# Jiang-Muyun/PointNet12

Hardware: NVIDIA B200
Metric: pointnet2_semseg_forward_points_per_sec (higher is better)
Workload: dtype f32 (MLP products as split bf16 hi/lo on tensor cores)

## Files before the change

### pointnet12_b200/csrc/fps.cu

```cuda
#include <cooperative_groups.h>

#include <type_traits>

#include "common.cuh"
#include "tcgen05.cuh"

namespace cg = cooperative_groups;

namespace pn {

constexpr int kMaxCluster = 16;
constexpr unsigned kNoIndex = 0xFFFFFFFFu;

struct __align__(32) FpsMsg {
    unsigned long long key;
    float x, y, z;
    float pad[3];
};

constexpr int kFpsSmemHeader = 2 * kMaxCluster * (int)sizeof(FpsMsg) + 2 * 32 * (int)sizeof(uint2) + 64;

__device__ __forceinline__ unsigned map_to_cta(unsigned addr, unsigned rank) {
    unsigned r;
    asm volatile("mapa.shared::cluster.u32 %0, %1, %2;" : "=r"(r) : "r"(addr), "r"(rank));
    return r;
}

template <int THREADS, int PTS, bool CLUSTER>
__global__ void __launch_bounds__(THREADS, 1)
fps_kernel(const float* __restrict__ xyz, int64_t sB, int64_t sN, int64_t sC, int N, int npoint,
           const int64_t* __restrict__ start, int64_t* __restrict__ out, unsigned long long* seq, int chunk, int async_x) {
    constexpr int NW = THREADS / 32;
    extern __shared__ __align__(32) unsigned char smem_raw[];
    FpsMsg* cl_slots = reinterpret_cast<FpsMsg*>(smem_raw);
    uint2* warp_slots = reinterpret_cast<uint2*>(smem_raw + 2 * kMaxCluster * sizeof(FpsMsg));
    unsigned long long* xbar = reinterpret_cast<unsigned long long*>(smem_raw + kFpsSmemHeader - 64);
    float* sx = reinterpret_cast<float*>(smem_raw + kFpsSmemHeader);
    float* sy = sx + chunk;
    float* sz = sy + chunk;

    unsigned CL = 1, rank = 0;
    if constexpr (CLUSTER) {
        cg::cluster_group cluster = cg::this_cluster();
        CL = cluster.num_blocks();
        rank = cluster.block_rank();
    }
    const int b = blockIdx.x / CL;
    const float* __restrict__ p = xyz + (int64_t)b * sB;
    const int base = rank * chunk;
    const int tid = threadIdx.x, lane = tid & 31, warp = tid >> 5;

    float x[PTS], y[PTS], z[PTS], d[PTS];
#pragma unroll
    for (int k = 0; k < PTS; ++k) {
        const int li = tid + k * THREADS;
        const int j = base + li;
        const bool ok = li < chunk && j < N;
        x[k] = ok ? p[(int64_t)j * sN] : 0.0f;
        y[k] = ok ? p[(int64_t)j * sN + sC] : 0.0f;
        z[k] = ok ? p[(int64_t)j * sN + 2 * sC] : 0.0f;
        d[k] = ok ? 1e10f : -2.0f;
        if (li < chunk) {
            sx[li] = x[k];
            sy[li] = y[k];
            sz[li] = z[k];
        }
    }
    int far = (int)start[b];
    float cx = p[(int64_t)far * sN], cy = p[(int64_t)far * sN + sC], cz = p[(int64_t)far * sN + 2 * sC];
    if constexpr (CLUSTER) {
        if (async_x && tid == 0) {
            tc::mbar_init(tc::smem_u32(&xbar[0]), 1);
            tc::mbar_init(tc::smem_u32(&xbar[1]), 1);
            tc::mbar_init_fence();
        }
        __syncthreads();
        cg::this_cluster().sync();
    } else {
        __syncthreads();
    }

    int64_t* __restrict__ o = out + (int64_t)b * npoint;
    for (int i = 0; i < npoint; ++i) {
        if (rank == 0 && tid == 0) {
            o[i] = far;
            if (seq) *reinterpret_cast<volatile unsigned long long*>(seq + (int64_t)b * npoint + i) = ((unsigned long long)(unsigned)far << 32) | 1ull;
        }
        float bv = -1.0f;
        int bk = 0;
#pragma unroll
        for (int k = 0; k < PTS; ++k) {
            const float dd = sqdist_diff(x[k], y[k], z[k], cx, cy, cz);
            d[k] = fminf(d[k], dd);
            if (d[k] > bv) {
                bv = d[k];
                bk = k;
            }
        }
        const unsigned vb = __float_as_uint(fmaxf(bv, 0.0f));
        const unsigned gi = bv < 0.0f ? kNoIndex : (unsigned)(base + tid + bk * THREADS);
        const unsigned wm = __reduce_max_sync(0xffffffffu, vb);
        const unsigned wi = __reduce_min_sync(0xffffffffu, vb == wm ? gi : kNoIndex);
        const int par = i & 1;
        unsigned bm, bi;
        if constexpr (NW > 1) {
            if (lane == 0) warp_slots[par * 32 + warp] = make_uint2(wm, wi);
            __syncthreads();
            const uint2 s = lane < NW ? warp_slots[par * 32 + lane] : make_uint2(0u, kNoIndex);
            bm = __reduce_max_sync(0xffffffffu, s.x);
            bi = __reduce_min_sync(0xffffffffu, s.x == bm ? s.y : kNoIndex);
        } else {
            bm = wm;
            bi = wi;
        }
        if constexpr (!CLUSTER) {
            far = (int)bi;
            cx = sx[far];
            cy = sy[far];
            cz = sz[far];
        } else {
            cg::cluster_group cluster = cg::this_cluster();
            if (async_x) {
                const unsigned l_bar = tc::smem_u32(&xbar[par]);
                if (tid == 0) tc::mbar_arrive_expect_tx(l_bar, CL * 20u);
                if (warp == 0 && lane < (int)CL) {
                    const unsigned long long key = ((unsigned long long)bm << 32) | (unsigned long long)(~bi);
                    const int li = bi == kNoIndex ? 0 : (int)bi - base;
                    const unsigned r_slot = map_to_cta(tc::smem_u32(&cl_slots[par * kMaxCluster + rank]), lane);
                    const unsigned r_bar = map_to_cta(l_bar, lane);
                    asm volatile(
                        "st.async.weak.shared::cluster.mbarrier::complete_tx::bytes.v4.b32 [%0], {%1, %2, %3, %4}, [%5];" ::"r"(r_slot),
                        "r"((unsigned)(key & 0xFFFFFFFFull)), "r"((unsigned)(key >> 32)), "r"(__float_as_uint(sx[li])),
                        "r"(__float_as_uint(sy[li])), "r"(r_bar)
                        : "memory");
                    asm volatile("st.async.weak.shared::cluster.mbarrier::complete_tx::bytes.b32 [%0], %1, [%2];" ::"r"(r_slot + 16),
                                 "r"(__float_as_uint(sz[li])), "r"(r_bar)
                                 : "memory");
                }
                tc::mbar_wait(l_bar, (unsigned)((i >> 1) & 1));
            } else {
            if (warp == 0 && lane < (int)CL) {
                FpsMsg m;
                m.key = ((unsigned long long)bm << 32) | (unsigned long long)(~bi);
                const int li = bi == kNoIndex ? 0 : (int)bi - base;
                m.x = sx[li];
                m.y = sy[li];
                m.z = sz[li];
                m.pad[0] = m.pad[1] = m.pad[2] = 0.0f;
                FpsMsg* dst = cluster.map_shared_rank(&cl_slots[par * kMaxCluster + rank], lane);
                *dst = m;
            }
            cluster.sync();
            }
            unsigned long long best = 0ull;
            int bc = 0;
            for (int c = 0; c < (int)CL; ++c) {
                const unsigned long long k = cl_slots[par * kMaxCluster + c].key;
                if (k > best) {
                    best = k;
                    bc = c;
                }
            }
            far = (int)(~(unsigned)(best & 0xFFFFFFFFull));
            const FpsMsg& w = cl_slots[par * kMaxCluster + bc];
            cx = w.x;
            cy = w.y;
            cz = w.z;
        }
    }
    if constexpr (CLUSTER) {
        if (async_x) cg::this_cluster().sync();
    }
}

struct __align__(32) FpsSlot {
    unsigned val, idx;
    float x, y, z;
    float pad[3];
};
constexpr int kMaxSlots = 64;
constexpr int kSlotBytes = 20;
constexpr int kAsyncSmemHeader = 64 + 2 * kMaxSlots * (int)sizeof(FpsSlot);

template <int NW, int PTS, bool ZT>
__global__ void __launch_bounds__(NW * 32, 1)
fps_async_kernel(const float* __restrict__ xyz, int64_t sB, int64_t sN, int64_t sC, int N, int npoint,
                 const int64_t* __restrict__ start, int64_t* __restrict__ out, unsigned long long* seq, int chunk) {
    constexpr int THREADS = NW * 32;
    extern __shared__ __align__(32) unsigned char smem_raw[];
    unsigned long long* mbar = reinterpret_cast<unsigned long long*>(smem_raw);
    FpsSlot* slots = reinterpret_cast<FpsSlot*>(smem_raw + 64);
    float* sx = reinterpret_cast<float*>(smem_raw + kAsyncSmemHeader);
    float* sy = sx + chunk;
    float* sz = sy + chunk;
    float* zt = sz + chunk;

    cg::cluster_group cluster = cg::this_cluster();
    const unsigned CL = cluster.num_blocks();
    const unsigned rank = cluster.block_rank();
    const int nslot = (int)CL * NW;
    const int b = blockIdx.x / CL;
    const float* __restrict__ p = xyz + (int64_t)b * sB;
    const int base = rank * chunk;
    const int tid = threadIdx.x, lane = tid & 31, warp = tid >> 5;

    static_assert(PTS % 2 == 0, "points are processed in packed pairs");
    unsigned long long xp[PTS / 2], yp[PTS / 2], zp[PTS / 2];
    float d[PTS];
#pragma unroll
    for (int k = 0; k < PTS; k += 2) {
        float x[2], y[2], z[2];
#pragma unroll
        for (int u = 0; u < 2; ++u) {
            const int li = tid + (k + u) * THREADS;
            const int j = base + li;
            const bool ok = li < chunk && j < N;
            x[u] = ok ? p[(int64_t)j * sN] : 0.0f;
            y[u] = ok ? p[(int64_t)j * sN + sC] : 0.0f;
            z[u] = ok ? p[(int64_t)j * sN + 2 * sC] : 0.0f;
            d[k + u] = ok ? 1e10f : -2.0f;
            if (li < chunk) {
                sx[li] = x[u];
                sy[li] = y[u];
                sz[li] = z[u];
            }
        }
        xp[k / 2] = pack2(x[0], x[1]);
        yp[k / 2] = pack2(y[0], y[1]);
        zp[k / 2] = pack2(z[0], z[1]);
    }
    if constexpr (ZT) {
        for (int i = tid; i < N; i += THREADS) zt[i] = p[(int64_t)i * sN + 2 * sC];
    }
    if (tid == 0) {
        tc::mbar_init(tc::smem_u32(&mbar[0]), 1);
        tc::mbar_init(tc::smem_u32(&mbar[1]), 1);
        tc::mbar_init_fence();
    }
    int far = (int)start[b];
    far = min(max(far, 0), N - 1);
    float cx = p[(int64_t)far * sN], cy = p[(int64_t)far * sN + sC], cz = p[(int64_t)far * sN + 2 * sC];
    __syncthreads();
    cluster.sync();

    const unsigned my_slot = rank * NW + warp;
    const unsigned dst_cta = lane < (int)CL ? lane : 0;
    const unsigned r_slot0 = map_to_cta(tc::smem_u32(&slots[my_slot]), dst_cta);
    const unsigned r_bar0 = map_to_cta(tc::smem_u32(&mbar[0]), dst_cta);
    const unsigned l_bar0 = tc::smem_u32(&mbar[0]);
    constexpr unsigned kParSlotOff = kMaxSlots * sizeof(FpsSlot), kParBarOff = sizeof(unsigned long long);

    int64_t* __restrict__ o = out + (int64_t)b * npoint;
    for (int i = 0; i < npoint; ++i) {
        const int par = i & 1;
        if (rank == 0 && tid == 0) {
            o[i] = far;
            if (seq) *reinterpret_cast<volatile unsigned long long*>(seq + (int64_t)b * npoint + i) = ((unsigned long long)(unsigned)far << 32) | 1ull;
        }
        if (i == npoint - 1) break;
        if (tid == 0)
            tc::mbar_arrive_expect_tx(l_bar0 + par * kParBarOff, (unsigned)(nslot * (ZT ? 16 : kSlotBytes)));
        float bv = -1.0f;
        int bk = 0;
        const unsigned long long ncx = pack2(-cx, -cx), ncy = pack2(-cy, -cy), ncz = pack2(-cz, -cz);
#pragma unroll
        for (int k = 0; k < PTS; k += 2) {
            float d0, d1;
            sqdist_diff2(xp[k / 2], yp[k / 2], zp[k / 2], ncx, ncy, ncz, d0, d1);
            d[k] = fminf(d[k], d0);
            if (d[k] > bv) {
                bv = d[k];
                bk = k;
            }
            d[k + 1] = fminf(d[k + 1], d1);
            if (d[k + 1] > bv) {
                bv = d[k + 1];
                bk = k + 1;
            }
        }
        const unsigned vb = __float_as_uint(fmaxf(bv, 0.0f));
        const unsigned gi = bv < 0.0f ? kNoIndex : (unsigned)(base + tid + bk * THREADS);
        const unsigned wm = __reduce_max_sync(0xffffffffu, vb);
        const unsigned wi = __reduce_min_sync(0xffffffffu, vb == wm ? gi : kNoIndex);
        if (lane < (int)CL) {
            const int li = wi == kNoIndex ? 0 : (int)wi - base;
            const float mx = sx[li], my = sy[li];
            const unsigned r_slot = r_slot0 + par * kParSlotOff, r_bar = r_bar0 + par * kParBarOff;
            asm volatile(
                "st.async.weak.shared::cluster.mbarrier::complete_tx::bytes.v4.b32 [%0], {%1, %2, %3, %4}, [%5];" ::"r"(
                    r_slot),
                "r"(wm), "r"(wi), "r"(__float_as_uint(mx)), "r"(__float_as_uint(my)), "r"(r_bar)
                : "memory");
            if constexpr (!ZT) {
                const float mz = sz[li];
                asm volatile("st.async.weak.shared::cluster.mbarrier::complete_tx::bytes.b32 [%0], %1, [%2];" ::"r"(
                                 r_slot + 16),
                             "r"(__float_as_uint(mz)), "r"(r_bar)
                             : "memory");
            }
        }
        tc::mbar_wait(l_bar0 + par * kParBarOff, (unsigned)((i >> 1) & 1));
        unsigned sv = 0u, si = kNoIndex;
        float px = 0.f, py = 0.f, pz = 0.f;
        if (lane < nslot) {
            const FpsSlot& s0 = slots[par * kMaxSlots + lane];
            sv = s0.val; si = s0.idx; px = s0.x; py = s0.y;
            if constexpr (!ZT) pz = s0.z;
        }
        if (lane + 32 < nslot) {
            const FpsSlot& s1 = slots[par * kMaxSlots + lane + 32];
            if (s1.val > sv || (s1.val == sv && s1.idx < si)) {
                sv = s1.val; si = s1.idx; px = s1.x; py = s1.y;
                if constexpr (!ZT) pz = s1.z;
            }
        }
        const unsigned bm = __reduce_max_sync(0xffffffffu, sv);
        const unsigned bi = __reduce_min_sync(0xffffffffu, sv == bm ? si : kNoIndex);
        const unsigned who = __ballot_sync(0xffffffffu, sv == bm && si == bi);
        const int src = __ffs(who) - 1;
        far = (int)bi;
        cx = __shfl_sync(0xffffffffu, px, src);
        cy = __shfl_sync(0xffffffffu, py, src);
        if constexpr (ZT) cz = zt[min(bi, (unsigned)(N - 1))];
        else cz = __shfl_sync(0xffffffffu, pz, src);
    }
    cluster.sync();
}

template <int NW, int PTS>
__global__ void __launch_bounds__(NW * 32, NW == 8 ? 2 : 1)
fps_pruned_kernel(const float* __restrict__ xyz, int64_t sB, int64_t sN, int64_t sC, const unsigned char* __restrict__ grid_ws,
                  size_t ws_stride, size_t sorted_off, int N, int npoint, const int64_t* __restrict__ start,
                  int64_t* __restrict__ out, unsigned long long* seq, int no_prune) {
    static_assert(PTS % 2 == 0, "points are processed in packed pairs");
    constexpr int CAP = NW * PTS * 32, NQ = PTS / 2;
    extern __shared__ __align__(32) unsigned char smem_raw[];
    unsigned long long* mbar = reinterpret_cast<unsigned long long*>(smem_raw);
    FpsSlot* slots = reinterpret_cast<FpsSlot*>(smem_raw + 64);
    float4* rec = reinterpret_cast<float4*>(smem_raw + kAsyncSmemHeader);

    cg::cluster_group cluster = cg::this_cluster();
    const unsigned CL = cluster.num_blocks();
    const unsigned rank = cluster.block_rank();
    const int nslot = (int)CL * NW;
    const int b = blockIdx.x / CL;
    const float* __restrict__ p = xyz + (int64_t)b * sB;
    const float4* __restrict__ sorted = reinterpret_cast<const float4*>(grid_ws + (size_t)b * ws_stride + sorted_off);
    const int tid = threadIdx.x, lane = tid & 31, warp = tid >> 5;
    float4* wrec = rec + (size_t)warp * NQ * 2 * 32 + lane;
    const int g0 = (int)rank * CAP + warp * PTS * 32;

    float d[PTS];
    float lo[3] = {3.0e38f, 3.0e38f, 3.0e38f}, hi[3] = {-3.0e38f, -3.0e38f, -3.0e38f};
#pragma unroll
    for (int q = 0; q < NQ; ++q) {
        float4 v[2];
#pragma unroll
        for (int u = 0; u < 2; ++u) {
            const int j = g0 + (2 * q + u) * 32 + lane;
            const bool ok = j < N;
            v[u] = make_float4(0.f, 0.f, 0.f, __int_as_float(-1));
            if (ok) v[u] = sorted[j];
            d[2 * q + u] = ok ? 1e10f : -2.0f;
            if (ok) {
                lo[0] = fminf(lo[0], v[u].x); hi[0] = fmaxf(hi[0], v[u].x);
                lo[1] = fminf(lo[1], v[u].y); hi[1] = fmaxf(hi[1], v[u].y);
                lo[2] = fminf(lo[2], v[u].z); hi[2] = fmaxf(hi[2], v[u].z);
            }
        }
        wrec[(q * 2 + 0) * 32] = make_float4(v[0].x, v[1].x, v[0].y, v[1].y);
        wrec[(q * 2 + 1) * 32] = make_float4(v[0].z, v[1].z, v[0].w, v[1].w);
    }
#pragma unroll
    for (int c = 0; c < 3; ++c)
#pragma unroll
        for (int o = 16; o; o >>= 1) {
            lo[c] = fminf(lo[c], __shfl_xor_sync(0xffffffffu, lo[c], o));
            hi[c] = fmaxf(hi[c], __shfl_xor_sync(0xffffffffu, hi[c], o));
        }
    const bool warp_empty = g0 >= N;
    if (tid == 0) {
        tc::mbar_init(tc::smem_u32(&mbar[0]), 1);
        tc::mbar_init(tc::smem_u32(&mbar[1]), 1);
        tc::mbar_init_fence();
    }
    int far = (int)start[b];
    far = min(max(far, 0), N - 1);
    float cx = p[(int64_t)far * sN], cy = p[(int64_t)far * sN + sC], cz = p[(int64_t)far * sN + 2 * sC];
    __syncthreads();
    cluster.sync();

    const unsigned my_slot = rank * NW + warp;
    const unsigned dst_cta = lane < (int)CL ? lane : 0;
    const unsigned r_slot0 = map_to_cta(tc::smem_u32(&slots[my_slot]), dst_cta);
    const unsigned r_bar0 = map_to_cta(tc::smem_u32(&mbar[0]), dst_cta);
    const unsigned l_bar0 = tc::smem_u32(&mbar[0]);
    constexpr unsigned kParSlotOff = kMaxSlots * sizeof(FpsSlot), kParBarOff = sizeof(unsigned long long);

    float wmax = warp_empty ? -1.0f : 1e10f;
    unsigned wm = 0u, wi = kNoIndex;
    float wx = 0.f, wy = 0.f, wz = 0.f;

    int64_t* __restrict__ o = out + (int64_t)b * npoint;
    for (int i = 0; i < npoint; ++i) {
        const int par = i & 1;
        if (rank == 0 && tid == 0) {
            o[i] = far;
            if (seq) *reinterpret_cast<volatile unsigned long long*>(seq + (int64_t)b * npoint + i) = ((unsigned long long)(unsigned)far << 32) | 1ull;
        }
        if (i == npoint - 1) break;
        if (tid == 0)
            tc::mbar_arrive_expect_tx(l_bar0 + par * kParBarOff, (unsigned)(nslot * kSlotBytes));
        const float ddx = fmaxf(fmaxf(__fsub_rn(lo[0], cx), __fsub_rn(cx, hi[0])), 0.0f);
        const float ddy = fmaxf(fmaxf(__fsub_rn(lo[1], cy), __fsub_rn(cy, hi[1])), 0.0f);
        const float ddz = fmaxf(fmaxf(__fsub_rn(lo[2], cz), __fsub_rn(cz, hi[2])), 0.0f);
        const float lb = __fadd_rn(__fadd_rn(__fmul_rn(ddx, ddx), __fmul_rn(ddy, ddy)), __fmul_rn(ddz, ddz));
        if (lb < wmax || (no_prune && !warp_empty)) {
            const unsigned long long ncx = pack2(-cx, -cx), ncy = pack2(-cy, -cy), ncz = pack2(-cz, -cz);
            float bv = -2.0f;
#pragma unroll
            for (int q = 0; q < NQ; ++q) {
                const float4 xy = wrec[(q * 2 + 0) * 32];
                const float4 zi = wrec[(q * 2 + 1) * 32];
                float d0, d1;
                sqdist_diff2(pack2(xy.x, xy.y), pack2(xy.z, xy.w), pack2(zi.x, zi.y), ncx, ncy, ncz, d0, d1);
                d[2 * q] = fminf(d[2 * q], d0);
                d[2 * q + 1] = fminf(d[2 * q + 1], d1);
                bv = fmaxf(bv, fmaxf(d[2 * q], d[2 * q + 1]));
            }
            const unsigned vb = __float_as_uint(fmaxf(bv, 0.0f));
            wm = __reduce_max_sync(0xffffffffu, vb);
            unsigned cand = kNoIndex;
            int kb = 0;
            if (bv >= 0.0f && vb == wm) {
#pragma unroll
                for (int k = 0; k < PTS; ++k) {
                    if (d[k] == bv) {
                        const float4 zi = wrec[((k >> 1) * 2 + 1) * 32];
                        const unsigned ov = __float_as_uint((k & 1) ? zi.w : zi.z);
                        if (ov < cand) {
                            cand = ov;
                            kb = k;
                        }
                    }
                }
            }
            wi = __reduce_min_sync(0xffffffffu, cand);
            const unsigned who = __ballot_sync(0xffffffffu, cand == wi && cand != kNoIndex);
            const int src = who ? __ffs(who) - 1 : 0;
            const float4 xy = wrec[((kb >> 1) * 2 + 0) * 32];
            const float4 zi = wrec[((kb >> 1) * 2 + 1) * 32];
            wx = __shfl_sync(0xffffffffu, (kb & 1) ? xy.y : xy.x, src);
            wy = __shfl_sync(0xffffffffu, (kb & 1) ? xy.w : xy.z, src);
            wz = __shfl_sync(0xffffffffu, (kb & 1) ? zi.y : zi.x, src);
            wmax = __uint_as_float(wm);
        }
        if (lane < (int)CL) {
            const unsigned r_slot = r_slot0 + par * kParSlotOff, r_bar = r_bar0 + par * kParBarOff;
            asm volatile(
                "st.async.weak.shared::cluster.mbarrier::complete_tx::bytes.v4.b32 [%0], {%1, %2, %3, %4}, [%5];" ::"r"(
                    r_slot),
                "r"(wm), "r"(wi), "r"(__float_as_uint(wx)), "r"(__float_as_uint(wy)), "r"(r_bar)
                : "memory");
            asm volatile("st.async.weak.shared::cluster.mbarrier::complete_tx::bytes.b32 [%0], %1, [%2];" ::"r"(r_slot + 16),
                         "r"(__float_as_uint(wz)), "r"(r_bar)
                         : "memory");
        }
        tc::mbar_wait(l_bar0 + par * kParBarOff, (unsigned)((i >> 1) & 1));
        unsigned sv = 0u, si = kNoIndex;
        float px = 0.f, py = 0.f, pz = 0.f;
        if (lane < nslot) {
            const FpsSlot& s0 = slots[par * kMaxSlots + lane];
            sv = s0.val; si = s0.idx; px = s0.x; py = s0.y; pz = s0.z;
        }
        if (lane + 32 < nslot) {
            const FpsSlot& s1 = slots[par * kMaxSlots + lane + 32];
            if (s1.val > sv || (s1.val == sv && s1.idx < si)) {
                sv = s1.val; si = s1.idx; px = s1.x; py = s1.y; pz = s1.z;
            }
        }
        const unsigned bm = __reduce_max_sync(0xffffffffu, sv);
        const unsigned bi = __reduce_min_sync(0xffffffffu, sv == bm ? si : kNoIndex);
        const unsigned who = __ballot_sync(0xffffffffu, sv == bm && si == bi);
        const int src = __ffs(who) - 1;
        far = (int)bi;
        cx = __shfl_sync(0xffffffffu, px, src);
        cy = __shfl_sync(0xffffffffu, py, src);
        cz = __shfl_sync(0xffffffffu, pz, src);
    }
    cluster.sync();
}

struct FpsCfg {
    int cluster = 0, threads = 0;
    int exchange = 0;
    bool no_ztable = false;
    bool query_only = false;
    bool block_async = true;
    int* ctas = nullptr;
    size_t* smem = nullptr;
};

template <typename Kern>
static int launch_cluster_kernel(Kern kern, const char* what, int CL, int threads, size_t smem, const FpsCfg& cfg_, const float* xyz,
                                 int64_t sB, int64_t sN, int64_t sC, int B, int N, int npoint, const int64_t* start, int64_t* out,
                                 unsigned long long* seq, int chunk, cudaStream_t stream) {
    if (cfg_.ctas) *cfg_.ctas = B * CL;
    if (cfg_.smem) *cfg_.smem = smem;
    if (cfg_.query_only) return PN_OK;
    cudaError_t e = cudaFuncSetAttribute(kern, cudaFuncAttributeMaxDynamicSharedMemorySize, (int)smem);
    if (e == cudaSuccess && CL > 8) e = cudaFuncSetAttribute(kern, cudaFuncAttributeNonPortableClusterSizeAllowed, 1);
    if (e != cudaSuccess) {
        cudaGetLastError();
        set_error("pn_fps_f32: cudaFuncSetAttribute failed: %s", cudaGetErrorString(e));
        return (int)e;
    }
    cudaLaunchConfig_t cfg = {};
    cfg.gridDim = dim3((unsigned)(B * CL));
    cfg.blockDim = dim3((unsigned)threads);
    cfg.dynamicSmemBytes = smem;
    cfg.stream = stream;
    cudaLaunchAttribute attr[1];
    if (CL > 1) {
        attr[0].id = cudaLaunchAttributeClusterDimension;
        attr[0].val.clusterDim.x = (unsigned)CL;
        attr[0].val.clusterDim.y = 1;
        attr[0].val.clusterDim.z = 1;
        cfg.attrs = attr;
        cfg.numAttrs = 1;
    }
    if constexpr (std::is_invocable_v<Kern, const float*, int64_t, int64_t, int64_t, int, int, const int64_t*, int64_t*, unsigned long long*, int, int>)
        e = cudaLaunchKernelEx(&cfg, kern, xyz, sB, sN, sC, N, npoint, start, out, seq, chunk, cfg_.block_async ? 1 : 0);
    else
        e = cudaLaunchKernelEx(&cfg, kern, xyz, sB, sN, sC, N, npoint, start, out, seq, chunk);
    if (e != cudaSuccess) {
        cudaGetLastError();
        set_error("pn_fps_f32: launch of %s failed (cluster=%d threads=%d smem=%zu): %s", what, CL, threads, smem,
                  cudaGetErrorString(e));
        return (int)e;
    }
    return PN_OK;
}

#define PN_FPS_ARGS fc, xyz, sB, sN, sC, B, N, npoint, start, out, seq, chunk, stream

template <int THREADS>
static int dispatch_barrier(int pts, int CL, const FpsCfg& fc, const float* xyz, int64_t sB, int64_t sN, int64_t sC, int B, int N, int npoint,
                            const int64_t* start, int64_t* out, unsigned long long* seq, int chunk, cudaStream_t stream) {
    const size_t smem = (size_t)kFpsSmemHeader + (size_t)chunk * 3 * sizeof(float);
#define PN_FPS_CASE(P)                                                                                              \
    if (pts <= P)                                                                                                   \
        return CL > 1 ? launch_cluster_kernel(fps_kernel<THREADS, P, true>, "fps_kernel", CL, THREADS, smem, PN_FPS_ARGS) \
                      : launch_cluster_kernel(fps_kernel<THREADS, P, false>, "fps_kernel", CL, THREADS, smem, PN_FPS_ARGS)
    PN_FPS_CASE(1);
    PN_FPS_CASE(2);
    PN_FPS_CASE(4);
    PN_FPS_CASE(8);
    if constexpr (THREADS <= 512) {
        PN_FPS_CASE(16);
    }
#undef PN_FPS_CASE
    set_error("pn_fps_f32: %d points per thread at %d threads exceeds the register-resident limit", pts, THREADS);
    return PN_ERR_UNSUPPORTED;
}

template <int NW>
static int dispatch_async(int pts, int CL, const FpsCfg& fc, const float* xyz, int64_t sB, int64_t sN, int64_t sC, int B, int N, int npoint,
                          const int64_t* start, int64_t* out, unsigned long long* seq, int chunk, cudaStream_t stream) {
    const size_t smem0 = (size_t)kAsyncSmemHeader + (size_t)chunk * 3 * sizeof(float);
    const bool zt = !fc.no_ztable && smem0 + (size_t)N * sizeof(float) <= 200 * 1024;
    const size_t smem = smem0 + (zt ? (size_t)N * sizeof(float) : 0);
#define PN_FPS_CASE(P)                                                                                                       \
    if (pts <= P)                                                                                                            \
        return zt ? launch_cluster_kernel(fps_async_kernel<NW, P, true>, "fps_async_kernel", CL, NW * 32, smem, PN_FPS_ARGS) \
                  : launch_cluster_kernel(fps_async_kernel<NW, P, false>, "fps_async_kernel", CL, NW * 32, smem, PN_FPS_ARGS)
    PN_FPS_CASE(4);
    PN_FPS_CASE(8);
    PN_FPS_CASE(12);
    PN_FPS_CASE(16);
    PN_FPS_CASE(24);
    PN_FPS_CASE(32);
    if constexpr (NW == 8) {
        PN_FPS_CASE(48);
    }
#undef PN_FPS_CASE
    set_error("pn_fps_f32: %d points per thread at %d warps exceeds the register-resident limit", pts, NW);
    return PN_ERR_UNSUPPORTED;
}

}

static int fps_cfg_from_opts(const pn_launch_opts* o, pn::FpsCfg* fc) {
    if (!o) return PN_OK;
    const int cluster_size = o->fps_cluster, threads = o->fps_threads, exchange = o->fps_exchange;
    const bool cl_ok = cluster_size == 0 || cluster_size == 1 || cluster_size == 2 || cluster_size == 3 || cluster_size == 4 ||
                       cluster_size == 8 || cluster_size == 16;
    const bool th_ok = threads == 0 || threads == 64 || threads == 128 || threads == 256 || threads == 512 ||
                       threads == 1024;
    PN_REQUIRE(cl_ok && th_ok && exchange >= 0 && exchange <= 3, PN_ERR_BAD_ARG,
               "pn_launch_opts: fps_cluster in {0,1,2,3,4,8,16}, fps_threads in {0,64..1024}, fps_exchange in {0,1,2,3}");
    fc->cluster = cluster_size;
    fc->threads = threads;
    fc->exchange = exchange == 3 ? 2 : exchange;
    fc->no_ztable = exchange == 3;
    fc->block_async = exchange != 1;
    return PN_OK;
}

static int fps_dispatch(const pn::FpsCfg& fc, const float* xyz, int64_t sB, int64_t sN, int64_t sC, int B, int N, int npoint,
                        const int64_t* start, int64_t* out, unsigned long long* seq, pn_stream_t stream_);

PN_EXPORT int pn_fps_f32(const float* xyz, int64_t sB, int64_t sN, int64_t sC, int B, int N, int npoint,
                         const int64_t* start, int64_t* out, const pn_launch_opts* opts, pn_stream_t stream_) {
    PN_REQUIRE(xyz && start && out, PN_ERR_BAD_ARG, "pn_fps_f32: null pointer");
    pn::FpsCfg fc;
    if (int rc = fps_cfg_from_opts(opts, &fc)) return rc;
    return fps_dispatch(fc, xyz, sB, sN, sC, B, N, npoint, start, out, nullptr, stream_);
}

PN_EXPORT int pn_fps_progress_f32(const float* xyz, int64_t sB, int64_t sN, int64_t sC, int B, int N, int npoint,
                                  const int64_t* start, int64_t* out, uint64_t* progress, const pn_launch_opts* opts,
                                  pn_stream_t stream_) {
    PN_REQUIRE(xyz && start && out && progress, PN_ERR_BAD_ARG, "pn_fps_progress_f32: null pointer");
    pn::FpsCfg fc;
    if (int rc = fps_cfg_from_opts(opts, &fc)) return rc;
    return fps_dispatch(fc, xyz, sB, sN, sC, B, N, npoint, start, out, reinterpret_cast<unsigned long long*>(progress), stream_);
}

PN_EXPORT int pn_fps_sorted_f32(const float* xyz, int64_t sB, int64_t sN, int64_t sC, const void* grid, size_t grid_bytes, int B,
                                int N, int npoint, const int64_t* start, int64_t* out, uint64_t* progress, const pn_launch_opts* opts,
                                pn_stream_t stream_) {
    using namespace pn;
    PN_REQUIRE(xyz && grid && start && out, PN_ERR_BAD_ARG, "pn_fps_sorted_f32: null pointer");
    PN_REQUIRE(B > 0 && N > 0 && npoint > 0, PN_ERR_BAD_ARG, "pn_fps_sorted_f32: B, N, npoint must be positive (got %d, %d, %d)", B, N,
               npoint);
    PN_REQUIRE(grid_bytes >= pn_ball_grid_bytes(B, N), PN_ERR_BAD_ARG, "pn_fps_sorted_f32: grid buffer too small");
    int NW = ((opts && opts->fps_threads == 512) || N > 2 * 12288) ? 16 : 32;
    if (opts && opts->fps_threads == 256 && N <= 8 * 6144) NW = 8;
    const int PTS = NW == 32 ? 12 : 24;
    const int CAP = NW * PTS * 32;
    const int CL = (int)ceil_div(N, CAP);
    PN_REQUIRE(CL <= 64 / NW, PN_ERR_UNSUPPORTED, "pn_fps_sorted_f32: N=%d exceeds %d (%d CTAs of %d points)", N, 64 / NW * CAP, 64 / NW, CAP);
    const int no_prune = (opts && opts->fps_exchange == 1) ? 1 : 0;
    auto launch = [&](auto kern) -> int {
        const size_t smem = (size_t)kAsyncSmemHeader + (size_t)CAP * sizeof(float4);
        cudaError_t e = cudaFuncSetAttribute(kern, cudaFuncAttributeMaxDynamicSharedMemorySize, (int)smem);
        if (e != cudaSuccess) {
            cudaGetLastError();
            set_error("pn_fps_sorted_f32: cudaFuncSetAttribute failed: %s", cudaGetErrorString(e));
            return (int)e;
        }
        cudaLaunchConfig_t cfg = {};
        cfg.gridDim = dim3((unsigned)(B * CL));
        cfg.blockDim = dim3((unsigned)(NW * 32));
        cfg.dynamicSmemBytes = smem;
        cfg.stream = (cudaStream_t)stream_;
        cudaLaunchAttribute attr[1];
        attr[0].id = cudaLaunchAttributeClusterDimension;
        attr[0].val.clusterDim.x = (unsigned)CL;
        attr[0].val.clusterDim.y = 1;
        attr[0].val.clusterDim.z = 1;
        cfg.attrs = attr;
        cfg.numAttrs = 1;
        e = cudaLaunchKernelEx(&cfg, kern, xyz, sB, sN, sC, static_cast<const unsigned char*>(grid), ball_grid_cloud_bytes(N),
                               ball_grid_sorted_offset(), N, npoint, start, out, reinterpret_cast<unsigned long long*>(progress),
                               no_prune);
        if (e != cudaSuccess) {
            cudaGetLastError();
            set_error("pn_fps_sorted_f32: launch failed (cluster=%d smem=%zu): %s", CL, smem, cudaGetErrorString(e));
            return (int)e;
        }
        return PN_OK;
    };
    return NW == 32 ? launch(fps_pruned_kernel<32, 12>) : (NW == 16 ? launch(fps_pruned_kernel<16, 24>) : launch(fps_pruned_kernel<8, 24>));
}

PN_EXPORT int pn_fps_launch_info(int B, int N, int npoint, const pn_launch_opts* opts, int* ctas, size_t* smem_bytes) {
    PN_REQUIRE(ctas && smem_bytes, PN_ERR_BAD_ARG, "pn_fps_launch_info: null pointer");
    pn::FpsCfg fc;
    if (int rc = fps_cfg_from_opts(opts, &fc)) return rc;
    fc.query_only = true;
    fc.ctas = ctas;
    fc.smem = smem_bytes;
    *ctas = 0;
    *smem_bytes = 0;
    return fps_dispatch(fc, reinterpret_cast<const float*>(16), 3 * (int64_t)N, 1, N, B, N, npoint,
                        reinterpret_cast<const int64_t*>(16), reinterpret_cast<int64_t*>(16), nullptr, nullptr);
}

static int fps_dispatch(const pn::FpsCfg& fc, const float* xyz, int64_t sB, int64_t sN, int64_t sC, int B, int N, int npoint,
                        const int64_t* start, int64_t* out, unsigned long long* seq, pn_stream_t stream_) {
    using namespace pn;
    PN_REQUIRE(B > 0 && N > 0 && npoint > 0, PN_ERR_BAD_ARG, "pn_fps_f32: B, N, npoint must be positive (got %d, %d, %d)", B,
               N, npoint);
    cudaStream_t stream = (cudaStream_t)stream_;
    int CL = fc.cluster;
    if (CL == 0) {
        if (N <= 3072) CL = 1;
        else if (N <= 6144) CL = 2;
        else if (N <= 12288) CL = 4;
        else if (N <= 65536) CL = 8;
        else CL = 16;
    }
    const int chunk = (int)ceil_div(N, CL);
    bool use_async = CL > 1 && fc.exchange != 1;
    int threads = fc.threads;
    if (use_async) {
        if (threads == 0) threads = (chunk <= 4096 && CL * 4 <= kMaxSlots) ? 128 : 256;
        const int nw = threads / 32;
        if (threads > 256 || CL * nw > kMaxSlots || ceil_div(chunk, threads) > (threads == 256 ? 48 : 32)) {
            PN_REQUIRE(fc.exchange != 2, PN_ERR_UNSUPPORTED,
                       "pn_fps_f32: st.async exchange needs cluster*warps <= 64, threads <= 256 and <= 32 (48 at 256 threads) points per thread "
                       "(N=%d cluster=%d threads=%d)", N, CL, threads);
            use_async = false;
            threads = fc.threads;
        }
    }
    if (use_async) {
        const int pts = (int)ceil_div(chunk, threads);
        PN_REQUIRE((size_t)kAsyncSmemHeader + (size_t)chunk * 12 <= 227 * 1024, PN_ERR_UNSUPPORTED,
                   "pn_fps_f32: N=%d needs %d points per CTA at cluster size %d; shared memory holds 19000", N, chunk, CL);
        switch (threads) {
            case 64: return dispatch_async<2>(pts, CL, PN_FPS_ARGS);
            case 128: return dispatch_async<4>(pts, CL, PN_FPS_ARGS);
            default: return dispatch_async<8>(pts, CL, PN_FPS_ARGS);
        }
    }
    if (threads == 0) threads = N <= 128 ? 64 : N <= 512 ? 128 : N <= 2048 ? 256 : 512;
    const int pts = (int)ceil_div(chunk, threads);
    PN_REQUIRE((size_t)kFpsSmemHeader + (size_t)chunk * 12 <= 227 * 1024, PN_ERR_UNSUPPORTED,
               "pn_fps_f32: N=%d needs %d points per CTA at cluster size %d; shared memory holds 19200", N, chunk, CL);
    switch (threads) {
        case 64: return dispatch_barrier<64>(pts, CL, PN_FPS_ARGS);
        case 128: return dispatch_barrier<128>(pts, CL, PN_FPS_ARGS);
        case 256: return dispatch_barrier<256>(pts, CL, PN_FPS_ARGS);
        case 512: return dispatch_barrier<512>(pts, CL, PN_FPS_ARGS);
        default: return dispatch_barrier<1024>(pts, CL, PN_FPS_ARGS);
    }
}
```

### pointnet12_b200/runtime.py

```python
from __future__ import annotations

import operator
import os
import time
from collections import deque
from typing import Dict, List, Optional, Tuple

import torch

from . import ops

_VERSION_OF = operator.attrgetter("_version")


class Ticket:

    __slots__ = ("set", "seq", "done", "to_host")

    def __init__(self, st, seq, done, to_host):
        self.set, self.seq, self.done, self.to_host = st, seq, done, to_host


class Pacer:

    def __init__(self, factor: float, window: int = 8, clock=time.perf_counter):
        self.factor, self.clock = float(factor), clock
        self.done_at = deque(maxlen=window)
        self.blocked = 0
        self.per_batch = None
        self.in_flight = 0
        self.last_submit = 0.0

    def next_submit_time(self) -> float:
        if self.in_flight <= 0:
            self.done_at.clear()
            self.blocked = 0
        return self.last_submit + self.factor * self.per_batch if self.per_batch is not None else 0.0

    def submitted(self) -> None:
        self.last_submit = self.clock()
        self.in_flight += 1

    def completed(self, waited: float) -> None:
        self.in_flight = max(0, self.in_flight - 1)
        self.blocked += waited > 20e-6
        self.done_at.append(self.clock())
        if len(self.done_at) == self.done_at.maxlen:
            seen = (self.done_at[-1] - self.done_at[0]) / (len(self.done_at) - 1)
            if self.per_batch is None:
                self.per_batch = seen
            elif self.blocked:
                self.per_batch = min(max(seen, 0.93 * self.per_batch), 1.05 * self.per_batch)
            else:
                self.per_batch *= 0.93
            self.done_at.clear()
            self.blocked = 0


class GraphedSemSeg:

    RING = 4
    FPS1_PIPELINED = (3, 256, 2)
    FPS1_DEEP = (2, 256, 2)

    def __init__(self, net, warmup: int = 2, depth: int = 1):
        self.net = net.module if hasattr(net, "module") else net
        self.warmup = warmup
        self.depth = max(1, int(depth))
        self.timing = False
        self._graphs: Dict[Tuple, dict] = {}
        self._tensors = list(self.net.parameters()) + list(self.net.buffers())
        self._sig, self._vsum, self._checks, self._last_check = None, 0, 0, 0.0
        self.pace = float(os.environ.get("PN12_PIPE_PACE", "0.92")) if self.depth > 1 else 0.0

    def _signature(self):
        return tuple((t.data_ptr(), t._version) for t in self._tensors)

    def _versions(self) -> int:
        return sum(map(_VERSION_OF, self._tensors))

    def _check_weights(self, dev):
        now = time.perf_counter()
        self._checks += 1
        full = self.depth == 1 or self._sig is None or now - self._last_check > 2e-3 or (self._checks & 63) == 0
        self._last_check = now
        if full:
            sig = self._signature()
            changed = sig != self._sig
        else:
            changed = self._versions() != self._vsum
            sig = self._signature() if changed else self._sig
        if changed:
            if self._graphs:
                torch.cuda.synchronize(dev)
                self._graphs.clear()
            self._sig, self._vsum = sig, self._versions()

    def _capture_options(self, st) -> dict:
        if self.depth == 1:
            return {"tile_counters": None}
        return {"tile_counters": st["counters"], "fps1_config": self.fps1_shape(st["x"].shape[2]), "stream_ball": False,
                "host_out_slices": int(os.environ.get("PN12_PIPE_HOST_SLICES", "1"))}

    def fps1_shape(self, N: int) -> Optional[Tuple[int, int, int]]:
        if self.depth == 1:
            return None
        first = self.FPS1_DEEP if self.depth >= 8 else self.FPS1_PIPELINED
        for cluster in (2, 3, 4, 8):
            if cluster >= first[0] and N <= cluster * 256 * 48:
                return (cluster, 256, 2)
        return None

    def _build_set(self, points: torch.Tensor, to_host: bool) -> dict:
        net, dev = self.net, points.device
        B, C, N = points.shape
        sizes = [N] + [m.npoint for m in (net.sa1, net.sa2, net.sa3)]
        st = {
            "x": torch.empty((B, C, N), dtype=torch.float32, device=dev),
            "starts": torch.zeros((len(sizes), B), dtype=torch.int64, device=dev),
            "sizes": sizes,
            "pinned": [torch.zeros((len(sizes), B), dtype=torch.int64).pin_memory() for _ in range(self.RING)],
            "events": [None] * self.RING,
            "ready": torch.cuda.Event(),
            "slot": 0,
            "stream": torch.cuda.Stream(dev),
            "counters": ops.TileCounters(dev, 128) if self.depth > 1 else None,
            "seq": -1,
        }
        st["x"].copy_(points)
        classes = net.conv2.out_channels
        labels = to_host == "labels"
        st["host_out"] = torch.empty((B, N, classes), dtype=torch.float32).pin_memory() if (to_host and not labels) else None
        st["host_labels"] = torch.empty((B, N), dtype=torch.uint8).pin_memory() if labels else None
        stream = st["stream"]
        stream.wait_stream(torch.cuda.current_stream(dev))
        with torch.cuda.stream(stream), torch.no_grad():
            for _ in range(self.warmup):
                with ops.options(**{k: v for k, v in self._capture_options(st).items() if k != "tile_counters"}):
                    net(st["x"], fps_starts=list(st["starts"].unbind(0)), host_out=st["host_out"])
        torch.cuda.current_stream(dev).wait_stream(stream)
        torch.cuda.synchronize(dev)
        graph = torch.cuda.CUDAGraph()
        with ops.options(**self._capture_options(st)):
            with torch.cuda.graph(graph, stream=stream), torch.no_grad():
                st["out"] = net(st["x"], fps_starts=list(st["starts"].unbind(0)), host_out=st["host_out"])
                if labels:
                    st["labels"] = ops.argmax_labels(st["out"])
                    st["host_labels"].copy_(st["labels"], non_blocking=True)
        st["graph"] = graph
        return st

    def _sets(self, points: torch.Tensor, dev, to_host) -> dict:
        self._check_weights(dev)
        mode = "labels" if to_host == "labels" else bool(to_host)
        key = (tuple(points.shape), dev, mode)
        entry = self._graphs.get(key)
        if entry is None:
            on_dev = points.to(dev)
            entry = self._graphs[key] = {"sets": [self._build_set(on_dev, mode) for _ in range(self.depth)], "n": 0,
                                           "pace": Pacer(self.pace)}
            for st in entry["sets"]:
                st["pace"] = entry["pace"]
            self._sig, self._vsum = self._signature(), self._versions()
        return entry

    @torch.no_grad()
    def submit(self, points: torch.Tensor, to_host=False) -> Ticket:
        dev = points.device if points.is_cuda else torch.device("cuda", torch.cuda.current_device())
        entry = self._sets(points, dev, to_host)
        if to_host and self.pace > 0.0:
            until = entry["pace"].next_submit_time()
            while True:
                rem = until - time.perf_counter()
                if rem <= 0.0:
                    break
                if rem > 150e-6:
                    time.sleep(rem - 100e-6)
            entry["pace"].submitted()
        seq = entry["n"]
        entry["n"] = seq + 1
        st = entry["sets"][seq % self.depth]
        st["seq"] = seq
        B = points.shape[0]
        slot = st["slot"] = (st["slot"] + 1) % self.RING
        ev = st["events"][slot]
        if ev is not None:
            ev.synchronize()
        else:
            ev = st["events"][slot] = torch.cuda.Event()
        pinned = st["pinned"][slot]
        for i, n in enumerate(st["sizes"]):
            torch.randint(0, n, (B,), dtype=torch.long, out=pinned[i])
        stream = st["stream"]
        ready = st["ready"]
        ready.record()
        stream.wait_event(ready)
        if points.is_cuda:
            points.record_stream(stream)
        with torch.cuda.stream(stream):
            st["starts"].copy_(pinned, non_blocking=True)
            ev.record()
            st["x"].copy_(points, non_blocking=True)
            st["graph"].replay()
            done = torch.cuda.Event(enable_timing=self.timing)
            done.record()
        return Ticket(st, seq, done, "labels" if to_host == "labels" else bool(to_host))

    def result(self, ticket: Ticket) -> torch.Tensor:
        if ticket.set["seq"] != ticket.seq:
            raise RuntimeError(f"the result of batch {ticket.seq} was overwritten: at most depth={self.depth} batches are in flight")
        if ticket.to_host:
            t0 = time.perf_counter()
            ticket.done.synchronize()
            if self.pace > 0.0:
                ticket.set["pace"].completed(time.perf_counter() - t0)
            return ticket.set["host_labels"] if ticket.to_host == "labels" else ticket.set["host_out"]
        torch.cuda.current_stream(ticket.set["out"].device).wait_event(ticket.done)
        return ticket.set["out"]

    @torch.no_grad()
    def __call__(self, points: torch.Tensor, out: torch.Tensor = None, to_host: bool = False) -> torch.Tensor:
        res = self.result(self.submit(points, to_host=to_host))
        if to_host:
            return res
        if out is not None:
            out.copy_(res, non_blocking=True)
            return out
        return res

    def run_pipelined(self, batches, to_host=False, consume=None) -> Optional[List[torch.Tensor]]:
        pending, results = [], []
        for k, pts in enumerate(batches):
            pending.append((k, self.submit(pts, to_host=to_host)))
            if len(pending) >= self.depth:
                j, t = pending.pop(0)
                r = self.result(t)
                results.append(consume(j, r) if consume is not None else r.clone())
        for j, t in pending:
            r = self.result(t)
            results.append(consume(j, r) if consume is not None else r.clone())
        return results


class GraphedModule:

    RING = 4

    def __init__(self, net, warmup: int = 2):
        self.net = net.module if hasattr(net, "module") else net
        self.warmup = warmup
        self._graphs: Dict[Tuple, dict] = {}
        self._tensors = list(self.net.parameters()) + list(self.net.buffers())
        self._sig = None

    def _signature(self):
        return tuple((t.data_ptr(), t._version) for t in self._tensors)

    def _forward(self, st):
        if st["starts"] is not None:
            return self.net(*st["in"], fps_starts=list(st["starts"].unbind(0)))
        return self.net(*st["in"])

    @torch.no_grad()
    def __call__(self, *inputs: torch.Tensor):
        dev = next((t.device for t in inputs if t.is_cuda), torch.device("cuda", torch.cuda.current_device()))
        sig = self._signature()
        if sig != self._sig:
            if self._graphs:
                torch.cuda.synchronize(dev)
                self._graphs.clear()
            self._sig = sig
        key = tuple((tuple(t.shape), t.dtype) for t in inputs) + (dev,)
        st = self._graphs.get(key)
        B = inputs[0].shape[0]
        if st is None:
            st = {"in": [torch.empty(t.shape, dtype=t.dtype, device=dev) for t in inputs], "starts": None, "slot": 0}
            sizes = self.net.fps_level_sizes(inputs[0].shape[2]) if hasattr(self.net, "fps_level_sizes") else []
            if sizes:
                st["sizes"] = sizes
                st["starts"] = torch.zeros((len(sizes), B), dtype=torch.int64, device=dev)
                st["pinned"] = [torch.zeros((len(sizes), B), dtype=torch.int64).pin_memory() for _ in range(self.RING)]
                st["events"] = [None] * self.RING
            for s, t in zip(st["in"], inputs):
                s.copy_(t)
            side = torch.cuda.Stream(dev)
            side.wait_stream(torch.cuda.current_stream(dev))
            with torch.cuda.stream(side):
                for _ in range(self.warmup):
                    self._forward(st)
            torch.cuda.current_stream(dev).wait_stream(side)
            torch.cuda.synchronize(dev)
            graph = torch.cuda.CUDAGraph()
            with torch.cuda.graph(graph):
                st["out"] = self._forward(st)
            st["graph"] = graph
            self._graphs[key] = st
            self._sig = self._signature()
        if st["starts"] is not None:
            slot = st["slot"] = (st["slot"] + 1) % self.RING
            if st["events"][slot] is not None:
                st["events"][slot].synchronize()
            pinned = st["pinned"][slot]
            for i, n in enumerate(st["sizes"]):
                pinned[i] = torch.randint(0, n, (B,), dtype=torch.long)
            st["starts"].copy_(pinned, non_blocking=True)
            ev = torch.cuda.Event()
            ev.record()
            st["events"][slot] = ev
        for s, t in zip(st["in"], inputs):
            s.copy_(t, non_blocking=True)
        st["graph"].replay()
        return st["out"]
```

Baseline: 492.1 million.

## Add bounding-box grouped FPS kernel that skips distance updates for far groups

```diff
diff --git a/pointnet12_b200/csrc/fps.cu b/pointnet12_b200/csrc/fps.cu
--- a/pointnet12_b200/csrc/fps.cu
+++ b/pointnet12_b200/csrc/fps.cu
@@ -491,6 +491,189 @@
     cluster.sync();
 }
 
+constexpr int kGroupNW = 8, kGroupPts = 48, kGroupSlots = 8, kGroups = kGroupPts / kGroupSlots;
+constexpr int kGroupCap = kGroupNW * 32 * kGroupPts;
+constexpr int kSlotBits = 14;
+static_assert(kGroupCap <= (1 << kSlotBits) && 2 * kGroupCap < (1 << (32 - kSlotBits)), "packed (index, slot) must fit 32 bits");
+
+__global__ void __launch_bounds__(kGroupNW * 32, 1)
+fps_groups_kernel(const float* __restrict__ xyz, int64_t sB, int64_t sN, int64_t sC, const unsigned char* __restrict__ grid_ws,
+                  size_t ws_stride, size_t sorted_off, int N, int npoint, const int64_t* __restrict__ start,
+                  int64_t* __restrict__ out, unsigned long long* seq) {
+    constexpr int NW = kGroupNW, PTS = kGroupPts, G = kGroupSlots;
+    extern __shared__ __align__(32) unsigned char smem_raw[];
+    unsigned long long* mbar = reinterpret_cast<unsigned long long*>(smem_raw);
+    FpsSlot* slots = reinterpret_cast<FpsSlot*>(smem_raw + 64);
+    float4* rec = reinterpret_cast<float4*>(smem_raw + kAsyncSmemHeader);
+    float4* box = rec + kGroupCap;
+
+    cg::cluster_group cluster = cg::this_cluster();
+    const unsigned CL = cluster.num_blocks();
+    const unsigned rank = cluster.block_rank();
+    const int nslot = (int)CL * NW;
+    const int b = blockIdx.x / CL;
+    const float* __restrict__ p = xyz + (int64_t)b * sB;
+    const float4* __restrict__ sorted = reinterpret_cast<const float4*>(grid_ws + (size_t)b * ws_stride + sorted_off);
+    const int tid = threadIdx.x, lane = tid & 31, warp = tid >> 5;
+    const int s0 = warp * PTS * 32;
+
+    unsigned long long xp[PTS / 2], yp[PTS / 2], zp[PTS / 2];
+    float d[PTS];
+    float gmax[kGroups];
+    unsigned pmin = kNoIndex;
+#pragma unroll
+    for (int g = 0; g < kGroups; ++g) {
+        float lo[3] = {3.0e38f, 3.0e38f, 3.0e38f}, hi[3] = {-3.0e38f, -3.0e38f, -3.0e38f};
+        gmax[g] = -2.0f;
+#pragma unroll
+        for (int k = g * G; k < (g + 1) * G; k += 2) {
+            float x[2], y[2], z[2];
+#pragma unroll
+            for (int u = 0; u < 2; ++u) {
+                const int s = s0 + (k + u) * 32 + lane;
+                const int j = ((g * NW + warp) * (int)CL + (int)rank) * (G * 32) + (k + u - g * G) * 32 + lane;
+                const bool ok = j < N;
+                const float4 v = ok ? sorted[j] : make_float4(0.f, 0.f, 0.f, 0.f);
+                const unsigned packed = ok ? ((unsigned)__float_as_int(v.w) << kSlotBits) | (unsigned)s : kNoIndex;
+                rec[s] = make_float4(v.x, v.y, v.z, __uint_as_float(packed));
+                x[u] = v.x;
+                y[u] = v.y;
+                z[u] = v.z;
+                d[k + u] = ok ? 1e10f : -2.0f;
+                if (ok) {
+                    lo[0] = fminf(lo[0], v.x); hi[0] = fmaxf(hi[0], v.x);
+                    lo[1] = fminf(lo[1], v.y); hi[1] = fmaxf(hi[1], v.y);
+                    lo[2] = fminf(lo[2], v.z); hi[2] = fmaxf(hi[2], v.z);
+                    gmax[g] = 1e10f;
+                    pmin = min(pmin, packed);
+                }
+            }
+            xp[k / 2] = pack2(x[0], x[1]);
+            yp[k / 2] = pack2(y[0], y[1]);
+            zp[k / 2] = pack2(z[0], z[1]);
+        }
+#pragma unroll
+        for (int c = 0; c < 3; ++c)
+#pragma unroll
+            for (int o = 16; o; o >>= 1) {
+                lo[c] = fminf(lo[c], __shfl_xor_sync(0xffffffffu, lo[c], o));
+                hi[c] = fmaxf(hi[c], __shfl_xor_sync(0xffffffffu, hi[c], o));
+            }
+        const float m = __uint_as_float(__reduce_max_sync(0xffffffffu, __float_as_uint(fmaxf(gmax[g], 0.0f))));
+        if (lane == g) {
+            box[(warp * kGroups + g) * 2 + 0] = make_float4(lo[0], lo[1], lo[2], m);
+            box[(warp * kGroups + g) * 2 + 1] = make_float4(hi[0], hi[1], hi[2], 0.f);
+        }
+    }
+    unsigned wi = __reduce_min_sync(0xffffffffu, pmin);
+    unsigned wm = wi == kNoIndex ? 0u : __float_as_uint(1e10f);
+    if (tid == 0) {
+        tc::mbar_init(tc::smem_u32(&mbar[0]), 1);
+        tc::mbar_init(tc::smem_u32(&mbar[1]), 1);
+        tc::mbar_init_fence();
+    }
+    int far = (int)start[b];
+    far = min(max(far, 0), N - 1);
+    float cx = p[(int64_t)far * sN], cy = p[(int64_t)far * sN + sC], cz = p[(int64_t)far * sN + 2 * sC];
+    __syncthreads();
+    cluster.sync();
+
+    const unsigned my_slot = rank * NW + warp;
+    const unsigned dst_cta = lane < (int)CL ? lane : 0;
+    const unsigned r_slot0 = map_to_cta(tc::smem_u32(&slots[my_slot]), dst_cta);
+    const unsigned r_bar0 = map_to_cta(tc::smem_u32(&mbar[0]), dst_cta);
+    const unsigned l_bar0 = tc::smem_u32(&mbar[0]);
+    constexpr unsigned kParSlotOff = kMaxSlots * sizeof(FpsSlot), kParBarOff = sizeof(unsigned long long);
+    const float4* lrec = rec + s0 + lane;
+    float4* wbox = box + warp * kGroups * 2;
+    const float4* lbox = wbox + min(lane, kGroups - 1) * 2;
+
+    int64_t* __restrict__ o = out + (int64_t)b * npoint;
+    for (int i = 0; i < npoint; ++i) {
+        const int par = i & 1;
+        if (rank == 0 && tid == 0) {
+            o[i] = far;
+            if (seq) *reinterpret_cast<volatile unsigned long long*>(seq + (int64_t)b * npoint + i) = ((unsigned long long)(unsigned)far << 32) | 1ull;
+        }
+        if (i == npoint - 1) break;
+        if (tid == 0)
+            tc::mbar_arrive_expect_tx(l_bar0 + par * kParBarOff, (unsigned)(nslot * kSlotBytes));
+        const float4 blo = lbox[0], bhi = lbox[1];
+        const float ddx = fmaxf(fmaxf(__fsub_rn(blo.x, cx), __fsub_rn(cx, bhi.x)), 0.0f);
+        const float ddy = fmaxf(fmaxf(__fsub_rn(blo.y, cy), __fsub_rn(cy, bhi.y)), 0.0f);
+        const float ddz = fmaxf(fmaxf(__fsub_rn(blo.z, cz), __fsub_rn(cz, bhi.z)), 0.0f);
+        const float lb = __fadd_rn(__fadd_rn(__fmul_rn(ddx, ddx), __fmul_rn(ddy, ddy)), __fmul_rn(ddz, ddz));
+        const unsigned upd = __ballot_sync(0xffffffffu, lb < blo.w) & ((1u << kGroups) - 1);
+        if (upd) {
+            const unsigned long long ncx = pack2(-cx, -cx), ncy = pack2(-cy, -cy), ncz = pack2(-cz, -cz);
+#pragma unroll
+            for (int g = 0; g < kGroups; ++g) {
+                if (!(upd & (1u << g))) continue;
+                float bv = -2.0f;
+#pragma unroll
+                for (int k = g * G; k < (g + 1) * G; k += 2) {
+                    float d0, d1;
+                    sqdist_diff2(xp[k / 2], yp[k / 2], zp[k / 2], ncx, ncy, ncz, d0, d1);
+                    d[k] = fminf(d[k], d0);
+                    d[k + 1] = fminf(d[k + 1], d1);
+                    bv = fmaxf(bv, fmaxf(d[k], d[k + 1]));
+                }
+                gmax[g] = bv;
+            }
+#pragma unroll
+            for (int g = 0; g < kGroups; ++g) {
+                if (!(upd & (1u << g))) continue;
+                const unsigned m = __reduce_max_sync(0xffffffffu, __float_as_uint(fmaxf(gmax[g], 0.0f)));
+                if (lane == 0) wbox[g * 2].w = __uint_as_float(m);
+            }
+            float bv = gmax[0];
+#pragma unroll
+            for (int g = 1; g < kGroups; ++g) bv = fmaxf(bv, gmax[g]);
+            const unsigned vb = __float_as_uint(fmaxf(bv, 0.0f));
+            wm = __reduce_max_sync(0xffffffffu, vb);
+            unsigned cand = kNoIndex;
+            if (bv >= 0.0f && vb == wm) {
+#pragma unroll
+                for (int g = 0; g < kGroups; ++g)
+                    if (gmax[g] == bv)
+#pragma unroll
+                        for (int k = g * G; k < (g + 1) * G; ++k)
+                            if (d[k] == bv) cand = min(cand, __float_as_uint(lrec[k * 32].w));
+            }
+            wi = __reduce_min_sync(0xffffffffu, cand);
+            __syncwarp();
+        }
+        if (lane < (int)CL) {
+            const float4 w = rec[wi == kNoIndex ? 0 : wi & ((1u << kSlotBits) - 1)];
+            const unsigned r_slot = r_slot0 + par * kParSlotOff, r_bar = r_bar0 + par * kParBarOff;
+            asm volatile(
+                "st.async.weak.shared::cluster.mbarrier::complete_tx::bytes.v4.b32 [%0], {%1, %2, %3, %4}, [%5];" ::"r"(
+                    r_slot),
+                "r"(wm), "r"(wi), "r"(__float_as_uint(w.x)), "r"(__float_as_uint(w.y)), "r"(r_bar)
+                : "memory");
+            asm volatile("st.async.weak.shared::cluster.mbarrier::complete_tx::bytes.b32 [%0], %1, [%2];" ::"r"(r_slot + 16),
+                         "r"(__float_as_uint(w.z)), "r"(r_bar)
+                         : "memory");
+        }
+        tc::mbar_wait(l_bar0 + par * kParBarOff, (unsigned)((i >> 1) & 1));
+        unsigned sv = 0u, si = kNoIndex;
+        float px = 0.f, py = 0.f, pz = 0.f;
+        if (lane < nslot) {
+            const FpsSlot& s = slots[par * kMaxSlots + lane];
+            sv = s.val; si = s.idx; px = s.x; py = s.y; pz = s.z;
+        }
+        const unsigned bm = __reduce_max_sync(0xffffffffu, sv);
+        const unsigned bi = __reduce_min_sync(0xffffffffu, sv == bm ? si : kNoIndex);
+        const unsigned who = __ballot_sync(0xffffffffu, sv == bm && si == bi);
+        const int src = __ffs(who) - 1;
+        far = (int)(bi >> kSlotBits);
+        cx = __shfl_sync(0xffffffffu, px, src);
+        cy = __shfl_sync(0xffffffffu, py, src);
+        cz = __shfl_sync(0xffffffffu, pz, src);
+    }
+    cluster.sync();
+}
+
 struct FpsCfg {
     int cluster = 0, threads = 0;
     int exchange = 0;
@@ -635,15 +818,8 @@
     PN_REQUIRE(B > 0 && N > 0 && npoint > 0, PN_ERR_BAD_ARG, "pn_fps_sorted_f32: B, N, npoint must be positive (got %d, %d, %d)", B, N,
                npoint);
     PN_REQUIRE(grid_bytes >= pn_ball_grid_bytes(B, N), PN_ERR_BAD_ARG, "pn_fps_sorted_f32: grid buffer too small");
-    int NW = ((opts && opts->fps_threads == 512) || N > 2 * 12288) ? 16 : 32;
-    if (opts && opts->fps_threads == 256 && N <= 8 * 6144) NW = 8;
-    const int PTS = NW == 32 ? 12 : 24;
-    const int CAP = NW * PTS * 32;
-    const int CL = (int)ceil_div(N, CAP);
-    PN_REQUIRE(CL <= 64 / NW, PN_ERR_UNSUPPORTED, "pn_fps_sorted_f32: N=%d exceeds %d (%d CTAs of %d points)", N, 64 / NW * CAP, 64 / NW, CAP);
-    const int no_prune = (opts && opts->fps_exchange == 1) ? 1 : 0;
-    auto launch = [&](auto kern) -> int {
-        const size_t smem = (size_t)kAsyncSmemHeader + (size_t)CAP * sizeof(float4);
+    auto launch = [&](auto kern, int CL, int NW, int records, auto... extra) -> int {
+        const size_t smem = (size_t)kAsyncSmemHeader + (size_t)records * sizeof(float4);
         cudaError_t e = cudaFuncSetAttribute(kern, cudaFuncAttributeMaxDynamicSharedMemorySize, (int)smem);
         if (e != cudaSuccess) {
             cudaGetLastError();
@@ -664,7 +840,7 @@
         cfg.numAttrs = 1;
         e = cudaLaunchKernelEx(&cfg, kern, xyz, sB, sN, sC, static_cast<const unsigned char*>(grid), ball_grid_cloud_bytes(N),
                                ball_grid_sorted_offset(), N, npoint, start, out, reinterpret_cast<unsigned long long*>(progress),
-                               no_prune);
+                               extra...);
         if (e != cudaSuccess) {
             cudaGetLastError();
             set_error("pn_fps_sorted_f32: launch failed (cluster=%d smem=%zu): %s", CL, smem, cudaGetErrorString(e));
@@ -672,7 +848,20 @@
         }
         return PN_OK;
     };
-    return NW == 32 ? launch(fps_pruned_kernel<32, 12>) : (NW == 16 ? launch(fps_pruned_kernel<16, 24>) : launch(fps_pruned_kernel<8, 24>));
+    if (opts && opts->fps_exchange == 2) {
+        PN_REQUIRE(N <= 2 * kGroupCap, PN_ERR_UNSUPPORTED, "pn_fps_sorted_f32: fps_exchange = 2 holds N <= %d points (got %d)",
+                   2 * kGroupCap, N);
+        return launch(fps_groups_kernel, (int)ceil_div(N, kGroupCap), kGroupNW, kGroupCap + 2 * kGroupNW * kGroups);
+    }
+    int NW = ((opts && opts->fps_threads == 512) || N > 2 * 12288) ? 16 : 32;
+    if (opts && opts->fps_threads == 256 && N <= 8 * 6144) NW = 8;
+    const int PTS = NW == 32 ? 12 : 24;
+    const int CAP = NW * PTS * 32;
+    const int CL = (int)ceil_div(N, CAP);
+    PN_REQUIRE(CL <= 64 / NW, PN_ERR_UNSUPPORTED, "pn_fps_sorted_f32: N=%d exceeds %d (%d CTAs of %d points)", N, 64 / NW * CAP, 64 / NW, CAP);
+    const int no_prune = (opts && opts->fps_exchange == 1) ? 1 : 0;
+    return NW == 32 ? launch(fps_pruned_kernel<32, 12>, CL, NW, CAP, no_prune)
+                    : (NW == 16 ? launch(fps_pruned_kernel<16, 24>, CL, NW, CAP, no_prune) : launch(fps_pruned_kernel<8, 24>, CL, NW, CAP, no_prune));
 }
 
 PN_EXPORT int pn_fps_launch_info(int B, int N, int npoint, const pn_launch_opts* opts, int* ctas, size_t* smem_bytes) {
diff --git a/pointnet12_b200/runtime.py b/pointnet12_b200/runtime.py
--- a/pointnet12_b200/runtime.py
+++ b/pointnet12_b200/runtime.py
@@ -62,6 +62,7 @@
     RING = 4
     FPS1_PIPELINED = (3, 256, 2)
     FPS1_DEEP = (2, 256, 2)
+    FPS1_GROUPS = (0, 256, 2)
 
     def __init__(self, net, warmup: int = 2, depth: int = 1):
         self.net = net.module if hasattr(net, "module") else net
@@ -99,7 +100,10 @@
     def _capture_options(self, st) -> dict:
         if self.depth == 1:
             return {"tile_counters": None}
-        return {"tile_counters": st["counters"], "fps1_config": self.fps1_shape(st["x"].shape[2]), "stream_ball": False,
+        N = st["x"].shape[2]
+        groups = ops.GRID_MIN_POINTS <= N <= 2 * 256 * 48
+        return {"tile_counters": st["counters"], "fps1_config": self.fps1_shape(N), "stream_ball": False,
+                "fps1_sorted": self.FPS1_GROUPS if groups else None,
                 "host_out_slices": int(os.environ.get("PN12_PIPE_HOST_SLICES", "1"))}
 
     def fps1_shape(self, N: int) -> Optional[Tuple[int, int, int]]:
```

New measurement: 482.1 million, median of 6. -2.0%, worse.
